# int-brain-lab/mtscomp

Measured on AMD Instinct MI355X. Metric: compress + decompress GB/s (raw int16), higher is better.
Workload: dtype int16

## Files before the change

### mtscomp_amd/csrc/match.hip

```cpp
#include <stdlib.h>

#include <type_traits>

#include "deflate_dev.h"

namespace mts {

__device__ __forceinline__ u32 prev_lane(u32 v, u32 first) { return (u32)__builtin_amdgcn_update_dpp((int)first, (int)v, 0x138, 0xf, 0xf, false); }
__device__ __forceinline__ u32 sel64(u64 mask, u32 a, u32 b)
{
    u32 r;
    asm("v_cndmask_b32_e64 %0, %1, %2, %3" : "=v"(r) : "v"(b), "v"(a), "s"(mask));
    return r;
}
__device__ __forceinline__ u32 and_xor(u32 a, u32 b, u32 c) { return __builtin_amdgcn_bitop3_b32(a, b, c, 0x60); }
__device__ __forceinline__ u64 make_entry(u32 rel, u32 lo, u32 hi)
{
    const u32 d = (((lo >> 5) & 0x3f) << 3) | (lo & 7);
    const u32 w0 = rel | (d << REL_BITS) | (((hi >> 24) & ((1u << (32 - REL_BITS - 9)) - 1)) << (REL_BITS + 9));
    const u32 w1 = (lo >> 24) | (hi << 8);
    return (u64)w0 | ((u64)w1 << 32);
}
__device__ __forceinline__ u32 lds_u32(const u32 *win, u32 addr)
{
    const u32 a = addr >> 2;
    return alignbyte(win[a + 1], win[a], addr & 3);
}

#ifndef MTS_M5_NT_KEYS
#define MTS_M5_NT_KEYS 0
#endif
#ifndef MTS_M5_STATS
#define MTS_M5_STATS 0
#endif
#ifndef MTS_M5_BIT_AND
#define MTS_M5_BIT_AND 0
#endif
#if MTS_M5_STATS
__device__ unsigned long long g_m5_stats[16];
#endif
constexpr int M5_WAVES = 8;
#ifndef MTS_M5_SX
#define MTS_M5_SX 1
#endif
#ifndef MTS_M5_WAVES
#define MTS_M5_WAVES (MTS_M5_SX == 1 ? 8 : MTS_M5_SX == 2 ? 9 : 10)
#endif
constexpr int M5W = MTS_M5_WAVES;
constexpr int M5_SLICES = 64;
constexpr int M6_SLICES = 64;
constexpr int M5_RING = 256;
constexpr int M5_ROWS = 32;
constexpr int M5_LEVELS = 4;
constexpr int M5_ROW_WORDS = M5_RING / 32 + 1;
constexpr int M5_TABLE = M5_ROWS * M5_ROW_WORDS * 4;
constexpr int M5_SLOTS = M5_LEVELS + 1;
constexpr int M5_SX_BYTES = MTS_M5_SX == 1 ? 8 : MTS_M5_SX == 2 ? 4 : 0;
constexpr int M5_WAVE_LDS = M5_RING * (8 + M5_SX_BYTES) + M5_SLOTS * M5_TABLE;
__device__ __forceinline__ constexpr int m5_slot(int d) { return d ? d + 1 : 0; }
#ifndef MTS_M5_LDS_PAD
#define MTS_M5_LDS_PAD 0
#endif
constexpr int M5_VLUT = 129 * 16;
constexpr int MATCH5_LDS = MTS_M5_LDS_PAD ? MTS_M5_LDS_PAD : (M5W * M5_WAVE_LDS + M5_VLUT > 56 * 1024 ? M5W * M5_WAVE_LDS + M5_VLUT : 56 * 1024);

__device__ __forceinline__ int m5_len04(u32 x1, bool &all4)
{
    u32 f;
    asm("v_ffbl_b32 %0, %1" : "=v"(f) : "v"(x1));
    all4 = f > 31;
    return (int)(f >> 3);
}
__device__ __forceinline__ u32 m5_mul24(u32 x, u32 c)
{
    u32 r;
    asm("v_mul_u32_u24 %0, %1, %2" : "=v"(r) : "v"(x), "v"(c));
    return r;
}
__device__ __forceinline__ u32 m5_hash24(u32 x) { return (m5_mul24(x, 0x9E3779u) >> 19) & 31; }
__device__ __forceinline__ u32 m5_ffbh(u32 x)
{
    u32 r;
    asm("v_ffbh_u32 %0, %1" : "=v"(r) : "v"(x));
    return r;
}
__device__ __forceinline__ u32 m5_off8(u32 z, u32 k)
{
    u32 r;
    asm("v_mad_i32_i24 %0, %1, -8, %2" : "=v"(r) : "v"(z), "v"(k));
    return r;
}
__device__ __forceinline__ void m5_keys(u32 e1, u32 (&k)[M5_LEVELS])
{
    const u32 p = m5_mul24(e1, 0x9E3779u);
    k[0] = (p >> 2) & 63;
    k[1] = (p >> 11) & 31;
    k[2] = (p >> 19) & 31;
    k[3] = m5_hash24(e1 ^ (e1 >> 11));
}

__global__ __launch_bounds__(M5W * 64) void k_match5(const u8 *__restrict__ stream, const TileDesc *__restrict__ tiles, int n_tiles, int nsl,
                                                          const u32 *__restrict__ sorted, u32 *__restrict__ tables, u32 *__restrict__ quarter, LevelCfg cfg,
                                                          u32 *__restrict__ flags, int all_quarters)
{
    extern __shared__ __attribute__((aligned(16))) u8 smem[];
    const u32 xcd = blockIdx.x & 7, jb = blockIdx.x >> 3;
    const u32 tile_id = (jb / (u32)nsl) * 8 + xcd, slice = jb % (u32)nsl;
    if (tile_id >= (u32)n_tiles) return;
    const TileDesc td = tiles[tile_id];
    const int wave = threadIdx.x >> 6, lane = threadIdx.x & 63;
    const u8 *gwin = stream + td.stream_off + td.w;
    auto wread = [&](u32 addr) -> u32 { return gld_u32_unaligned(gwin, addr); };
    u64 *SE = (u64 *)(smem + wave * (M5_RING * 8));
    u64 *SX = (u64 *)(smem + M5W * M5_RING * 8 + wave * (M5_RING * 8));
    u32 *TB = (u32 *)(smem + M5W * M5_RING * (8 + M5_SX_BYTES) + M5_VLUT + wave * (M5_SLOTS * M5_TABLE));
    const uint4 *VLUT = (const uint4 *)(smem + M5W * M5_RING * (8 + M5_SX_BYTES));
    typedef __attribute__((address_space(3))) const u64 *lds_u64p;
    const u32 se_base = (u32)(size_t)(__attribute__((address_space(3))) u8 *)(u8 *)SE;
    if (se_base & (M5_RING * 8 - 1)) __builtin_trap();
    auto ring_e = [&](u32 o8) -> u64 { return *(lds_u64p)(size_t)((o8 & (M5_RING * 8 - 8)) | se_base); };
#if MTS_M5_SX == 2
    typedef __attribute__((address_space(3))) const u32 *lds_u32p;
    auto ring_x = [&](u32 o8) -> u32 { return *(lds_u32p)(size_t)((((o8 & (M5_RING * 8 - 8)) | se_base) >> 1) + M5W * M5_RING * 8); };
#else
    auto ring_x = [&](u32 o8) -> u64 { return *(lds_u64p)(size_t)(((o8 & (M5_RING * 8 - 8)) | se_base) + M5W * M5_RING * 8); };
#endif
    u32 *T = tables + td.stream_off, *TQ = quarter + td.stream_off;
    u32 *sink = flags + MATCH_SINK_WORD0 + (blockIdx.x & (MATCH_SINK_LINES - 1)) * MATCH_SINK_LINE_WORDS + (threadIdx.x & 63);
    if (threadIdx.x < 2 && slice == 0) {
        const u32 hashed_end = td.w + td.wlen;
        const u32 p = hashed_end + threadIdx.x;
        if (p >= td.a && p < td.own_end) { T[p] = 0; if (all_quarters) TQ[p] = 0; }
    }
    if (td.wlen == 0) return;
    const u32 *sk = sorted + td.sorted_off;
    const u32 wlen = td.wlen, n = td.n;
    const u32 ngroups = (wlen + 63) / 64;
    const u32 halo = td.a - td.w;
    const u32 chain = (u32)cfg.chain, qchain = (u32)cfg.chain >> 2;
    const u32 nwv = (u32)nsl * M5W;
    const u32 gpw = (ngroups + nwv - 1) / nwv;
    const u32 g_begin = (slice * M5W + wave) * gpw, g_end = min(ngroups, g_begin + gpw);
#if MTS_M5_NT_KEYS
    auto slot_rel = [&](int idx) -> u32 { return __builtin_nontemporal_load(&sk[idx < 0 ? 0 : (u32)idx < wlen ? (u32)idx : wlen - 1]) & REL_MASK; };
#else
    auto slot_rel = [&](int idx) -> u32 { return sk[idx < 0 ? 0 : (u32)idx < wlen ? (u32)idx : wlen - 1] & REL_MASK; };
#endif
#if MTS_M5_NT_KEYS
    auto slot_fwd = [&](u32 idx) -> u32 { return __builtin_nontemporal_load(&sk[min(idx, wlen - 1)]) & REL_MASK; };
#else
    auto slot_fwd = [&](u32 idx) -> u32 { return sk[min(idx, wlen - 1)] & REL_MASK; };
#endif
    const int i_first = (int)g_begin * 64 + lane;
    const u32 r_ha = slot_rel(i_first - 128), r_hb = slot_rel(i_first - 64), r_0 = slot_rel(i_first), r_1 = slot_rel(i_first + 64);
    for (int k = threadIdx.x; k <= 128; k += M5W * 64) {
        uint4 v;
        v.w = k >= 32 ? 0xffffffffu : k ? 0xffffffffu << (32 - k) : 0u;
        v.z = k >= 64 ? 0xffffffffu : k > 32 ? 0xffffffffu << (64 - k) : 0u;
        v.y = k >= 96 ? 0xffffffffu : k > 64 ? 0xffffffffu << (96 - k) : 0u;
        v.x = k >= 128 ? 0xffffffffu : k > 96 ? 0xffffffffu << (128 - k) : 0u;
        ((uint4 *)(smem + M5W * M5_RING * (8 + M5_SX_BYTES)))[k] = v;
    }
    __syncthreads();
    if (g_begin >= g_end) return;
    for (int k = lane; k < M5_SLOTS * M5_TABLE / 16; k += 64) ((uint4 *)TB)[k] = make_uint4(0, 0, 0, 0);
    __builtin_amdgcn_wave_barrier();
    u32 h_carry = 0xffffffffu;
#if MTS_M5_STATS
    u32 st_groups = 0, st_r1 = 0, st_r2 = 0, st_s1 = 0, st_s2 = 0;
    u64 st_t[6] = {0, 0, 0, 0, 0, 0};
    u64 st_mark = 0;
#define M5_MARK(k) do { if (MTS_M5_STATS == 2) { const u64 t_ = (u64)clock64(); st_t[k] += t_ - st_mark; st_mark = t_; } } while (0)
#endif
    u32 rc_carry = 0;
    u32 run_carry = 0;
    const u32 le_lo = lane >= 31 ? 0xffffffffu : (2u << lane) - 1, le_hi = lane < 32 ? 0u : lane == 63 ? 0xffffffffu : (2u << (lane - 32)) - 1;
    u32 inv[6];
#pragma unroll
    for (int j = 0; j < 6; j++) inv[j] = ((lane >> j) & 1) ? 0u : 0xffffffffu;
    auto commit = [&](int idx, u32 rc, u32 lo, u32 hi, u64 x, u32 (&key)[M5_LEVELS], u32 &nbv, u64 &vm) -> u64 {
        const u32 rp = (u32)idx & (M5_RING - 1), word = rp >> 5, bit = 1u << (rp & 31);
        const bool valid = (u32)idx < wlen;
        vm = ballot64(valid);
        const u64 ce = valid ? make_entry(rc, lo, hi) : ~0ull;
        const u32 h = valid ? hash_of(lo) : 0xfffffffeu;
        const u32 hp = prev_lane(h, h_carry), rcp = prev_lane(rc, rc_carry);
        const u64 sr = ballot64(h != hp);
        if (vm & ~sr & ballot64(rc <= rcp)) { if (lane == 0) atomicOr(flags, 1u); }
        h_carry = (u32)__builtin_amdgcn_readlane((int)h, 63);
        rc_carry = (u32)__builtin_amdgcn_readlane((int)rc, 63);
        if (__builtin_popcountll(sr) <= 6) {
            nbv = (u32)lane + run_carry;
            for (u64 m = sr; m; m &= m - 1) { const u32 d = (u32)lane - (u32)__builtin_ctzll(m); nbv = d < nbv ? d : nbv; }
        } else {
            const u32 mlo = (u32)sr & le_lo, mhi = (u32)(sr >> 32) & le_hi;
            const u32 top = mhi ? 63u - (u32)__builtin_clz(mhi) : 31u - (u32)__builtin_clz(mlo | 1u);
            nbv = (mlo | mhi) ? (u32)lane - top : (u32)lane + run_carry;
        }
        nbv = nbv < 128u ? nbv : 128u;
        run_carry = sr ? (u32)__builtin_clzll(sr) + 1u : (run_carry + 64u < 128u ? run_carry + 64u : 128u);
        m5_keys((u32)(ce >> 32), key);
        const u32 wp = word & ~1u;
        {
            u32 *t1 = TB + 2 * (M5_TABLE / 4) + lane * M5_ROW_WORDS + wp;
            t1[0] = 0; t1[1] = 0;
            if (lane < 32) { t1[64 * M5_ROW_WORDS] = 0; t1[64 * M5_ROW_WORDS + 1] = 0; }
            u32 m0 = (u32)vm, m1 = (u32)(vm >> 32);
#pragma unroll
            for (int j = 0; j < 6; j++) {
#if MTS_M5_BIT_AND
                u32 t;
                asm volatile("v_and_b32 %0, %1, %2" : "=v"(t) : "n"(1 << j), "v"(key[0]));
                const u64 B = ballot64(t != 0);
#else
                const u64 B = ballot64((key[0] >> j) & 1);
#endif
                m0 = and_xor(m0, (u32)B, inv[j]); m1 = and_xor(m1, (u32)(B >> 32), inv[j]);
            }
            { u32 *t0 = TB + lane * M5_ROW_WORDS + wp; t0[0] = m0; t0[1] = m1; }
        }
        __builtin_amdgcn_wave_barrier();
#pragma unroll
        for (int d = 1; d < M5_LEVELS; d++)
            if (valid) atomicOr(&TB[m5_slot(d) * (M5_TABLE / 4) + key[d] * M5_ROW_WORDS + word], bit);
        SE[rp] = ce;
#if MTS_M5_SX == 1
        SX[rp] = x;
#elif MTS_M5_SX == 2
        ((u32 *)(smem + M5W * M5_RING * 8))[wave * M5_RING + rp] = (u32)x;
#endif
        return ce;
    };
    typedef u32 u32x4_a4 __attribute__((ext_vector_type(4), aligned(4)));
    auto load16 = [&](u32 r, u32 &lo, u32 &hi, u64 &x) {
        const u8 *q = gwin + (r & ~3u);
        const u32x4_a4 w = *(const u32x4_a4 *)q;
        lo = alignbyte(w.y, w.x, r);
        hi = alignbyte(w.z, w.y, r);
        const u32 b8 = alignbyte(w.w, w.z, r), b12 = alignbyte(0u, w.w, r);
        x = (u64)__builtin_amdgcn_alignbit(b8, hi, 24) | ((u64)(__builtin_amdgcn_alignbit(b12, b8, 24) & 0xffffu) << 32);
    };
    u32 rc_c = r_0, rc_n = r_1;
    u32 lo_c, hi_c;
    u64 x_c;
    {
        u32 kk[M5_LEVELS], nb;
        u64 vmm;
        const u32 ra = r_ha, rb = r_hb;
        u32 la, ha, lb, hb;
        u64 xa, xb;
        load16(ra, la, ha, xa);
        load16(rb, lb, hb, xb);
        load16(rc_c, lo_c, hi_c, x_c);
        *sink = 0;
        commit(i_first - 128, ra, la, ha, xa, kk, nb, vmm);
        __builtin_amdgcn_wave_barrier();
        commit(i_first - 64, rb, lb, hb, xb, kk, nb, vmm);
    }
    for (u32 g = g_begin; g < g_end; g++) {
        const u32 i0 = g * 64, i = i0 + lane;
        u32 key[M5_LEVELS], nbv;
        __builtin_amdgcn_wave_barrier();
#if MTS_M5_STATS == 2
        st_mark = (u64)clock64();
#endif
        u64 vm;
        const u64 e = commit((int)i, rc_c, lo_c, hi_c, x_c, key, nbv, vm);
        const u64 ex = x_c;
        __builtin_amdgcn_wave_barrier();
        rc_c = rc_n;
        load16(rc_c, lo_c, hi_c, x_c);
        rc_n = slot_fwd(i + 128);
        const u32 e0 = (u32)e, e1 = (u32)(e >> 32);
        const u32 rel_p = e0 & REL_MASK;
        const bool own = i < wlen && rel_p >= halo;
        const u64 ownm = vm & ballot64(rel_p >= halo);
#if MTS_M5_STATS == 2
        if (!ownm) { *sink = 0; M5_MARK(5); continue; }
        M5_MARK(0);
#else
        if (!ownm) { *sink = 0; continue; }
#endif
        const u32 p_abs = td.w + rel_p;
        const u32 look = n - p_abs;
        const u32 maxlen = look < (u32)MAX_MATCH ? look : (u32)MAX_MATCH;
        const u32 nice = (u32)cfg.nice < look ? (u32)cfg.nice : look;
        const int lim1 = (int)(p_abs > (u32)MAX_DIST + 1 ? p_abs - MAX_DIST - 1 : 0) - (int)td.w;
        const int limn = (int)(p_abs > (u32)MAX_DIST ? p_abs - MAX_DIST : 0) - (int)td.w;
        const u32 lo = (i + 128) & (M5_RING - 1), w0 = lo >> 5, sh = lo & 31, lo8 = lo << 3;
        nbv = own ? (nbv < chain ? nbv : chain) : 0;
        u32 V[4], A4[4], A5[4], A6[4], A7[4];
        {
            const uint4 v = VLUT[nbv];
            V[0] = v.x; V[1] = v.y; V[2] = v.z; V[3] = v.w;
        }
        auto rowmask = [&](const int d, const u32 (&in)[4], u32 (&out)[4]) __attribute__((always_inline)) {
            const u8 *row = (const u8 *)(TB + m5_slot(d) * (M5_TABLE / 4) + key[d] * M5_ROW_WORDS);
            auto word = [&](const u32 k) -> u32 { return *(const u32 *)(row + (((w0 + k) << 2) & 28u)); };
            const u32 W0 = word(0), W1 = word(1), W2 = word(2), W3 = word(3), W4 = word(4);
            out[0] = in[0] & __builtin_amdgcn_alignbit(W1, W0, sh);
            out[1] = in[1] & __builtin_amdgcn_alignbit(W2, W1, sh);
            out[2] = in[2] & __builtin_amdgcn_alignbit(W3, W2, sh);
            out[3] = in[3] & __builtin_amdgcn_alignbit(W4, W3, sh);
        };
        rowmask(0, V, A4);
        rowmask(1, A4, A5);
        rowmask(2, A5, A6);
        rowmask(3, A6, A7);
#if MTS_M5_STATS == 2
        asm volatile("" :: "v"(A7[0]), "v"(A7[1]), "v"(A7[2]), "v"(A7[3]));
        M5_MARK(1);
#endif
        int best = -1, qbest = -1;
        u32 bdist = 0, qdist = 0;
        asm volatile("" : "+v"(best), "+v"(bdist));
        auto walks = [&](auto near_end) __attribute__((always_inline)) {
        constexpr bool NEAR_END = decltype(near_end)::value;
        auto set_stop = [&]() {
#pragma unroll
            for (int w = 0; w < 4; w++) { A4[w] = 0; A5[w] = 0; A6[w] = 0; A7[w] = 0; }
        };
        auto cand = [&](const u32 o8 , const u32 c0, const u32 c1, const u32 rel_c, auto &&narrow, auto &&finish) __attribute__((always_inline)) {
            const u32 x0 = (c0 ^ e0) >> REL_BITS, x1 = c1 ^ e1;
            if ((x0 & 0x1ff) == 0) {
                bool all4;
                int len = m5_len04(x1, all4);
                if (all4) len = 4;
                if (all4 && (x0 >> 9) == 0) {
#if MTS_M5_SX == 1
                    const u64 y = ring_x(o8) ^ ex;
                    const u32 len0 = 13;
#elif MTS_M5_SX == 2
                    const u32 y = ring_x(o8) ^ (u32)ex;
                    const u32 len0 = 11;
#else
                    const u32 y = wread(rel_c + 7) ^ (u32)ex;
                    const u32 len0 = 11;
#endif
                    if (y) len = 4 + (int)((u32)__builtin_ctzll((u64)y) >> 3);
                    else {
                        const u32 cap = NEAR_END ? maxlen : (u32)MAX_MATCH;
                        u32 full = len0;
                        while (full < cap) {
                            const u32 x = wread(rel_c + full) ^ wread(rel_p + full);
                            if (x) { full += (u32)__builtin_ctz(x) >> 3; break; }
                            full += 4;
                        }
                        full = full < cap ? full : cap;
                        len = (int)full - 3;
                        if (!NEAR_END && full >= (u32)cfg.nice) { best = len; bdist = rel_p - rel_c; set_stop(); finish(); }
                    }
                }
                if (NEAR_END) len = len < (int)maxlen - 3 ? len : (int)maxlen - 3;
                if (len > best) {
                    best = len; bdist = rel_p - rel_c;
                    narrow();
                    if (NEAR_END && len >= (int)nice - 3) { set_stop(); finish(); }
                }
            }
        };
        auto walk = [&](const u32 tb, const u32 &m0, const u32 &m1, const u32 &m2, const u32 &m3, const u32 &m4, const u32 part, const bool head) __attribute__((always_inline)) {
            auto pick = [&]() -> u32 {
                u32 r = best >= 0 ? m1 : m0;
                asm volatile("" : "+v"(r));
                r = best >= 1 ? m2 : r;
                asm volatile("" : "+v"(r));
                r = best >= 2 ? m3 : r;
                asm volatile("" : "+v"(r));
                return best >= 3 ? m4 : r;
            };
            auto pick_longer = [&]() -> u32 {
                u32 r = best >= 1 ? m2 : m1;
                asm volatile("" : "+v"(r));
                r = best >= 2 ? m3 : r;
                asm volatile("" : "+v"(r));
                return best >= 3 ? m4 : r;
            };
            u32 el = head ? m0 & part : pick() & part;
            if (head) {
#if MTS_M5_STATS
                st_r1++; st_s1 += (u32)__popcll(ballot64(el != 0));
#endif
                const u32 o8 = lo8 + 127 * 8;
                const u64 c = ring_e(o8);
                if ((int)el < 0) {
                    el &= 0x7fffffffu;
                    const u32 c0 = (u32)c, c1 = (u32)(c >> 32);
                    const u32 rel_c = c0 & REL_MASK;
                    if ((int)rel_c > lim1) cand(o8, c0, c1, rel_c, [&]() { el &= pick_longer(); }, [&]() { el = 0; });
                    else el = 0;
                }
            }
            while (any64(el != 0)) {
#if MTS_M5_STATS
                st_r1++; st_s1 += (u32)__popcll(ballot64(el != 0));
#endif
                {
                    const bool had = el != 0;
                    const u32 z = m5_ffbh(el);
                    const u32 t = tb + 31 - z;
                    const u32 o8 = m5_off8(z, lo8 + ((tb + 31) << 3));
                    const u64 c = ring_e(o8);
                    const u32 c0 = (u32)c, c1 = (u32)(c >> 32);
                    const u32 rel_c = c0 & REL_MASK;
                    const bool in_range = had && (int)rel_c > ((!head && t == 127) ? lim1 : limn);
                    u32 rm = in_range ? 0xffffffffu : 0u;
                    asm volatile("" : "+v"(rm));
                    el = el & ~(0x80000000u >> (z & 31)) & rm;
                    if (in_range) cand(o8, c0, c1, rel_c, [&]() { el &= pick_longer(); }, [&]() { el = 0; });
                }
            }
        };
        const u32 qpart = qchain >= 32 ? 0xffffffffu : ~(0xffffffffu >> qchain);
#define MTS_WALK(w, part, head) walk(32 * (w), V[w], A4[w], A5[w], A6[w], A7[w], part, head)
        MTS_WALK(3, qpart, true);
        qbest = best; qdist = bdist;
        if (qpart != 0xffffffffu) MTS_WALK(3, ~qpart, false);
#undef MTS_WALK
#if MTS_M5_STATS == 2
        M5_MARK(2);
#endif
        {
            auto pickw = [&](const int w) __attribute__((always_inline)) -> u32 {
                u32 r = best >= 1 ? A5[w] : A4[w];
                asm volatile("" : "+v"(r));
                r = best >= 2 ? A6[w] : r;
                asm volatile("" : "+v"(r));
                return best >= 3 ? A7[w] : r;
            };
            const u64 c3 = ballot64(best >= 0), c4 = ballot64(best >= 1), c5 = ballot64(best >= 2), c6 = ballot64(best >= 3);
            auto pick0 = [&](const int w) __attribute__((always_inline)) -> u32 {
                u32 r = sel64(c3, A4[w], V[w]);
                r = sel64(c4, A5[w], r);
                r = sel64(c5, A6[w], r);
                return sel64(c6, A7[w], r);
            };
            u32 f2 = pick0(2), f1 = pick0(1), f0 = pick0(0);
            u32 ko2 = lo8 + ((64 + 31) << 3), ko1 = lo8 + ((32 + 31) << 3), ko0 = lo8 + (31 << 3);
            asm volatile("" : "+v"(ko2), "+v"(ko1), "+v"(ko0));
            while (any64((f2 | f1 | f0) != 0)) {
#if MTS_M5_STATS
                st_r2++; st_s2 += (u32)__popcll(ballot64((f2 | f1 | f0) != 0));
#endif
                if (f2 | f1 | f0) {
                    const bool t2 = f2 != 0, t1 = f1 != 0;
                    const u32 cur = t2 ? f2 : t1 ? f1 : f0;
                    const u32 tbo = t2 ? ko2 : t1 ? ko1 : ko0;
                    const u32 z = (u32)__builtin_clz(cur);
                    const u32 o8 = m5_off8(z, tbo);
                    const u64 c = ring_e(o8);
                    const u32 c0 = (u32)c, c1 = (u32)(c >> 32);
                    const u32 rel_c = c0 & REL_MASK;
                    const bool in_range = (int)rel_c > limn;
                    u32 rm = in_range ? 0xffffffffu : 0u;
                    asm volatile("" : "+v"(rm));
                    const u32 ncur = cur & ~(0x80000000u >> z);
                    f2 = (t2 ? ncur : f2) & rm;
                    f1 = ((!t2 && t1) ? ncur : f1) & rm;
                    f0 = ((!t2 && !t1) ? ncur : f0) & rm;
                    if (in_range) cand(o8, c0, c1, rel_c, [&]() { f2 &= pickw(2); f1 &= pickw(1); f0 &= pickw(0); }, [&]() { f2 = 0; f1 = 0; f0 = 0; });
                }
            }
        }
        };
        if (ownm & ballot64(look < (u32)MAX_MATCH)) walks(std::true_type{}); else walks(std::false_type{});
#if MTS_M5_STATS == 2
        M5_MARK(3);
#endif
        {
            const u32 f = bdist | ((u32)(best > 0 ? best : 0) << 15), q = qdist | ((u32)(qbest > 0 ? qbest : 0) << 15);
            u32 e = f;
            const bool differ = q != f, side = differ && qbest > (int)cfg.good - 3;
            if (differ) e |= side ? TE_QSIDE : TE_QNONE;
            if (own && (side || all_quarters)) TQ[p_abs] = q;
            u32 *dst = own ? T + p_abs : sink;
            *dst = e;
        }
#if MTS_M5_STATS
        st_groups++;
#if MTS_M5_STATS == 2
        M5_MARK(4);
#endif
#endif
    }
#if MTS_M5_STATS
    if (lane == 0) { atomicAdd(&g_m5_stats[0], st_groups); atomicAdd(&g_m5_stats[1], st_r1); atomicAdd(&g_m5_stats[2], st_r2); atomicAdd(&g_m5_stats[3], st_s1); atomicAdd(&g_m5_stats[4], st_s2); for (int k = 0; k < 6; k++) atomicAdd(&g_m5_stats[5 + k], st_t[k]); }
#endif
}

constexpr int M6_RING = 1024;
constexpr int M6_ROW_WORDS = M6_RING / 32 + 1;
constexpr int M6_TABLE = M5_ROWS * M6_ROW_WORDS * 4;
constexpr int MATCH6_LDS = 2 * M6_RING * 8 + M5_SLOTS * M6_TABLE + M5_VLUT;

__global__ __launch_bounds__(M5_WAVES * 64) void k_match6(const u8 *__restrict__ stream, const TileDesc *__restrict__ tiles, int n_tiles, int nsl,
                                                          const u32 *__restrict__ sorted, u32 *__restrict__ tables, u32 *__restrict__ quarter, LevelCfg cfg,
                                                          u32 *__restrict__ flags, int all_quarters)
{
    extern __shared__ __attribute__((aligned(16))) u8 smem[];
    __shared__ u32 wg_h[M5_WAVES], wg_rc[M5_WAVES], wg_tail[M5_WAVES], wg_min;
    const u32 xcd = blockIdx.x & 7, jb = blockIdx.x >> 3;
    const u32 tile_id = (jb / (u32)nsl) * 8 + xcd, slice = jb % (u32)nsl;
    if (tile_id >= (u32)n_tiles) return;
    const TileDesc td = tiles[tile_id];
    const int wave = threadIdx.x >> 6, lane = threadIdx.x & 63;
    const u8 *gwin = stream + td.stream_off + td.w;
    auto wread = [&](u32 addr) -> u32 { return gld_u32_unaligned(gwin, addr); };
    u64 *SE = (u64 *)smem;
    u64 *SX = SE + M6_RING;
    u32 *TB = (u32 *)(smem + 2 * M6_RING * 8);
    u32 *T = tables + td.stream_off, *TQ = quarter + td.stream_off;
    if (threadIdx.x < 2 && slice == 0) {
        const u32 hashed_end = td.w + td.wlen;
        const u32 p = hashed_end + threadIdx.x;
        if (p >= td.a && p < td.own_end) { T[p] = 0; if (all_quarters) TQ[p] = 0; }
    }
    if (td.wlen == 0) return;
    const u32 *sk = sorted + td.sorted_off;
    const u32 wlen = td.wlen, n = td.n;
    const u32 ngroups = (wlen + 63) / 64;
    const u32 halo = td.a - td.w;
    const u32 chain = (u32)cfg.chain, qchain = (u32)cfg.chain >> 2;
    const u32 gpb = ((ngroups + (u32)nsl - 1) / (u32)nsl + M5_WAVES - 1) / M5_WAVES * M5_WAVES;
    const u32 gb_begin = slice * gpb, gb_end = min(ngroups, gb_begin + gpb);
    if (gb_begin >= gb_end) return;
    for (int k = threadIdx.x; k < M5_SLOTS * M6_TABLE / 4; k += M5_WAVES * 64) TB[k] = 0;
    const uint4 *VLUT = (const uint4 *)(smem + 2 * M6_RING * 8 + M5_SLOTS * M6_TABLE);
    for (int k = threadIdx.x; k <= 128; k += M5_WAVES * 64) {
        uint4 v;
        v.w = k >= 32 ? 0xffffffffu : k ? 0xffffffffu << (32 - k) : 0u;
        v.z = k >= 64 ? 0xffffffffu : k > 32 ? 0xffffffffu << (64 - k) : 0u;
        v.y = k >= 96 ? 0xffffffffu : k > 64 ? 0xffffffffu << (96 - k) : 0u;
        v.x = k >= 128 ? 0xffffffffu : k > 96 ? 0xffffffffu << (128 - k) : 0u;
        ((uint4 *)(smem + 2 * M6_RING * 8 + M5_SLOTS * M6_TABLE))[k] = v;
    }
    u32 inv[6];
#pragma unroll
    for (int j = 0; j < 6; j++) inv[j] = ((lane >> j) & 1) ? 0u : 0xffffffffu;
    typedef u32 u32x4_a4 __attribute__((ext_vector_type(4), aligned(4)));
    auto load16 = [&](u32 r, u32 &lo, u32 &hi, u64 &x) {
        const u8 *q = gwin + (r & ~3u);
        const u32x4_a4 w = *(const u32x4_a4 *)q;
        lo = alignbyte(w.y, w.x, r);
        hi = alignbyte(w.z, w.y, r);
        const u32 b8 = alignbyte(w.w, w.z, r), b12 = alignbyte(0u, w.w, r) & 0xffu;
        x = (u64)(hi >> 24) | ((u64)b8 << 8) | ((u64)b12 << 40);
    };
    struct Batch { bool valid; u32 rc, lo, hi; u64 x; };
    auto fetch = [&](int idx0, Batch &bt) {
        const int idx = idx0 + lane;
        bt.valid = idx >= 0 && (u32)idx < wlen;
        bt.rc = bt.valid ? sk[idx] & REL_MASK : 0;
        load16(bt.rc, bt.lo, bt.hi, bt.x);
    };
    auto commit = [&](int idx0, const Batch &bt) {
        const u32 rp = (u32)(idx0 + lane) & (M6_RING - 1), word = rp >> 5, bit = 1u << (rp & 31);
        const u64 ce = bt.valid ? make_entry(bt.rc, bt.lo, bt.hi) : ~0ull;
        u32 key[M5_LEVELS];
        m5_keys((u32)(ce >> 32), key);
        const u32 wp = word & ~1u;
        u32 *t1 = TB + 2 * (M6_TABLE / 4) + lane * M6_ROW_WORDS + wp;
        t1[0] = 0; t1[1] = 0;
        if (lane < 32) { t1[64 * M6_ROW_WORDS] = 0; t1[64 * M6_ROW_WORDS + 1] = 0; }
        const u64 vm = ballot64(bt.valid);
        u32 m0 = (u32)vm, m1 = (u32)(vm >> 32);
#pragma unroll
        for (int j = 0; j < 6; j++) {
            const u64 B = ballot64((key[0] >> j) & 1);
            m0 = and_xor(m0, (u32)B, inv[j]); m1 = and_xor(m1, (u32)(B >> 32), inv[j]);
        }
        { u32 *t0 = TB + lane * M6_ROW_WORDS + wp; t0[0] = m0; t0[1] = m1; }
        __builtin_amdgcn_wave_barrier();
#pragma unroll
        for (int d = 1; d < M5_LEVELS; d++)
            if (bt.valid) atomicOr(&TB[m5_slot(d) * (M6_TABLE / 4) + key[d] * M6_ROW_WORDS + word], bit);
        SE[rp] = ce;
        SX[rp] = bt.x;
    };
    u32 c_h = 0xfffffffdu, c_rc = 0, c_tail = 0;
    if (gb_begin > 0) {
        const u32 i1 = gb_begin * 64 - 1;
        c_rc = sk[i1] & REL_MASK;
        c_h = hash_of(wread(c_rc));
        if (threadIdx.x == 0) wg_min = 0xffffffffu;
        __syncthreads();
        for (u32 r = 0; r * (M5_WAVES * 64) < chain; r++) {
            const u32 t = 1 + threadIdx.x + r * (M5_WAVES * 64);
            const bool mism = t > i1 || hash_of(wread(sk[i1 - (t > i1 ? 0 : t)] & REL_MASK)) != c_h;
            if (mism) atomicMin(&wg_min, t);
            __syncthreads();
            const u32 found = wg_min;
            __syncthreads();
            if (found != 0xffffffffu) break;
        }
        c_tail = wg_min < chain ? wg_min : chain;
        __syncthreads();
    }
    for (u32 gs = gb_begin; gs < gb_end; gs += M5_WAVES) {
        const int G0 = (int)gs * 64;
        const u32 g = gs + (u32)wave;
        const bool active = g < gb_end;
        const u32 i = g * 64 + lane;
        const u32 rp0 = (active && i < wlen) ? sk[i] & REL_MASK : 0;
        u32 own_lo, own_hi;
        u64 ex;
        load16(rp0, own_lo, own_hi, ex);
        Batch ba, bb;
        fetch(G0 - 128 + 64 * wave, ba);
        if (wave < 2) fetch(G0 - 128 + 64 * (wave + 8), bb);
        const u64 e = make_entry(rp0, own_lo, own_hi);
        const u32 e0 = (u32)e, e1 = (u32)(e >> 32);
        const u32 rel_p = e0 & REL_MASK;
        const bool own = active && i < wlen && rel_p >= halo;
        u32 key[M5_LEVELS];
        m5_keys(e1, key);
        const u32 p_abs = td.w + rel_p;
        const u32 look = n - p_abs;
        const u32 maxlen = look < (u32)MAX_MATCH ? look : (u32)MAX_MATCH;
        const u32 nice = (u32)cfg.nice < look ? (u32)cfg.nice : look;
        const int lim1 = (int)(p_abs > (u32)MAX_DIST + 1 ? p_abs - MAX_DIST - 1 : 0) - (int)td.w;
        const int limn = (int)(p_abs > (u32)MAX_DIST ? p_abs - MAX_DIST : 0) - (int)td.w;
        u32 best = 2, bdist = 0, qbest = 2, qdist = 0;
        bool stop = false, qtaken = false;
        const bool have = active && i < wlen;
        const u32 h_own = have ? hash_of(own_lo) : 0xfffffffeu;
        if (lane == 63) { wg_h[wave] = h_own; wg_rc[wave] = rel_p; }
        __syncthreads();
        commit(G0 - 128 + 64 * wave, ba);
        if (wave < 2) commit(G0 - 128 + 64 * (wave + 8), bb);
        u32 nbv;
        {
            u32 hp = __shfl_up(h_own, 1, 64), rcp = __shfl_up(rel_p, 1, 64);
            if (lane == 0) { hp = wave ? wg_h[wave - 1] : c_h; rcp = wave ? wg_rc[wave - 1] : c_rc; }
            const bool starts_run = h_own != hp;
            if (any64(have && !starts_run && rel_p <= rcp)) { if (lane == 0) atomicOr(flags, 1u); }
            const u64 sr = ballot64(starts_run);
            if (lane == 0) wg_tail[wave] = sr ? (u32)__builtin_clzll(sr) + 1u : 0u;
            __syncthreads();
            u32 t = c_tail;
            for (int w = 0; w < wave; w++) { const u32 x = wg_tail[w]; t = x ? x : (t + 64u < chain ? t + 64u : chain); }
            const u32 le_lo = lane >= 31 ? 0xffffffffu : (2u << lane) - 1, le_hi = lane < 32 ? 0u : lane == 63 ? 0xffffffffu : (2u << (lane - 32)) - 1;
            const u32 mlo = (u32)sr & le_lo, mhi = (u32)(sr >> 32) & le_hi;
            const u32 top = mhi ? 63u - (u32)__builtin_clz(mhi) : 31u - (u32)__builtin_clz(mlo | 1u);
            nbv = (mlo | mhi) ? (u32)lane - top : (u32)lane + t;
            nbv = own ? (nbv < chain ? nbv : chain) : 0;
            u32 tt = c_tail;
            for (int w = 0; w < M5_WAVES; w++) { const u32 x = wg_tail[w]; tt = x ? x : (tt + 64u < chain ? tt + 64u : chain); }
            c_tail = tt; c_h = wg_h[M5_WAVES - 1]; c_rc = wg_rc[M5_WAVES - 1];
        }
        if (wave < 2) fetch(G0 - 256 + 64 * wave, ba);
        for (u32 jbase = 0, blk = 0;; jbase += 128, blk++) {
            if ((u32)(wave >> 1) == (blk & 3)) commit(G0 - (int)jbase - 256 + 64 * (wave & 1), ba);
            if ((u32)(wave >> 1) == ((blk + 1) & 3)) fetch(G0 - (int)jbase - 384 + 64 * (wave & 1), ba);
            if (jbase == qchain && !qtaken) { qbest = best; qdist = bdist; qtaken = true; }
            const u32 nbl = nbv > jbase ? (nbv - jbase < 128 ? nbv - jbase : 128) : 0;
            if (any64(nbl != 0 && !stop)) {
                const u32 lo = (u32)((int)i - (int)jbase - 128) & (M6_RING - 1), w0 = lo >> 5, sh = lo & 31;
                u32 V[4], A4[4], A5[4], A6[4], A7[4];
                {
                    const uint4 v = VLUT[nbl];
                    V[0] = v.x; V[1] = v.y; V[2] = v.z; V[3] = v.w;
                }
                auto rowmask = [&](const int d, const u32 (&in)[4], u32 (&out)[4]) __attribute__((always_inline)) {
                    const u8 *row = (const u8 *)(TB + m5_slot(d) * (M6_TABLE / 4) + key[d] * M6_ROW_WORDS);
                    auto word = [&](const u32 k) -> u32 { return *(const u32 *)(row + (((w0 + k) << 2) & 124u)); };
                    const u32 W0 = word(0), W1 = word(1), W2 = word(2), W3 = word(3), W4 = word(4);
                    out[0] = in[0] & __builtin_amdgcn_alignbit(W1, W0, sh);
                    out[1] = in[1] & __builtin_amdgcn_alignbit(W2, W1, sh);
                    out[2] = in[2] & __builtin_amdgcn_alignbit(W3, W2, sh);
                    out[3] = in[3] & __builtin_amdgcn_alignbit(W4, W3, sh);
                };
                rowmask(0, V, A4);
                rowmask(1, A4, A5);
                rowmask(2, A5, A6);
                rowmask(3, A6, A7);
                auto pickw = [&](const int w) __attribute__((always_inline)) -> u32 {
                    u32 r = best >= 3 ? A4[w] : V[w];
                    asm volatile("" : "+v"(r));
                    r = best >= 4 ? A5[w] : r;
                    asm volatile("" : "+v"(r));
                    r = best >= 5 ? A6[w] : r;
                    asm volatile("" : "+v"(r));
                    return best >= 6 ? A7[w] : r;
                };
                const bool first = jbase == 0;
                auto walk = [&](const bool u3, const bool u2, const bool u1, const bool u0) __attribute__((always_inline)) {
                    u32 f3 = (stop || !u3) ? 0u : pickw(3), f2 = (stop || !u2) ? 0u : pickw(2);
                    u32 f1 = (stop || !u1) ? 0u : pickw(1), f0 = (stop || !u0) ? 0u : pickw(0);
                    while (any64((f3 | f2 | f1 | f0) != 0)) {
                        if (f3 | f2 | f1 | f0) {
                            const bool t3 = f3 != 0, t2 = f2 != 0, t1 = f1 != 0;
                            const u32 cur = t3 ? f3 : t2 ? f2 : t1 ? f1 : f0;
                            const u32 tb = t3 ? 96u : t2 ? 64u : t1 ? 32u : 0u;
                            const u32 z = (u32)__builtin_clz(cur);
                            const u32 ncur = cur & ~(0x80000000u >> z);
                            f3 = t3 ? ncur : f3;
                            f2 = (!t3 && t2) ? ncur : f2;
                            f1 = (!t3 && !t2 && t1) ? ncur : f1;
                            f0 = (!t3 && !t2 && !t1) ? ncur : f0;
                            const u32 t = tb + 31 - z;
                            const u32 slot = (lo + t) & (M6_RING - 1);
                            const u64 c = SE[slot];
                            const u32 c0 = (u32)c, c1 = (u32)(c >> 32);
                            const u32 rel_c = c0 & REL_MASK;
                            if ((int)rel_c > ((first && t == 127) ? lim1 : limn)) {
                                const u32 x0 = (c0 ^ e0) >> REL_BITS, x1 = c1 ^ e1;
                                if ((x0 & 0x1ff) == 0) {
                                    u32 len = x1 ? 3 + ((u32)__builtin_ctz(x1) >> 3) : 7;
                                    if (x1 == 0 && (x0 >> 9) == 0) {
                                        const u64 y = SX[slot] ^ ex;
                                        if (y) len = 7 + ((u32)__builtin_ctzll(y) >> 3);
                                        else {
                                            len = 13;
                                            while (len < maxlen) {
                                                const u32 x = wread(rel_c + len) ^ wread(rel_p + len);
                                                if (x) { len += (u32)__builtin_ctz(x) >> 3; break; }
                                                len += 4;
                                            }
                                        }
                                    }
                                    len = len < maxlen ? len : maxlen;
                                    if (len > best) {
                                        best = len; bdist = rel_p - rel_c;
                                        if (len >= nice) stop = true;
                                        f3 &= pickw(3); f2 &= pickw(2); f1 &= pickw(1); f0 &= pickw(0);
                                    }
                                }
                            } else stop = true;
                            if (stop) { f3 = 0; f2 = 0; f1 = 0; f0 = 0; }
                        }
                    }
                };
                if (first && qchain == 64) {
                    walk(true, true, false, false);
                    qbest = best; qdist = bdist; qtaken = true;
                    walk(false, false, true, true);
                } else walk(true, true, true, true);
            } else if (jbase == 0 && qchain == 64) { qbest = best; qdist = bdist; qtaken = true; }
            if (!__syncthreads_or(!stop && nbv > jbase + 128)) break;
        }
        if (!qtaken) { qbest = best; qdist = bdist; }
        if (own) te_store(T, TQ, p_abs, best, bdist, qbest, qdist, (u32)cfg.good, all_quarters);
    }
}

int launch_match(hipStream_t st, const u8 *d_stream, const TileDesc *d_tiles, int n_tiles, const u32 *d_sorted, u32 *d_tables, u32 *d_quarter,
                 LevelCfg cfg, u32 *d_flags, int all_quarters)
{
    if (n_tiles == 0) return MTS_OK;
    if (cfg.chain <= 128) {
        if (MATCH5_LDS > 65536) MTS_LDS_ATTR(k_match5, MATCH5_LDS);
        int nsl = M5_SLICES;
        if (const char *e = getenv("MTS_MATCH_SLICES")) nsl = atoi(e) > 0 ? atoi(e) : nsl;
        const int grid = (n_tiles + 7) / 8 * 8 * nsl;
        hipLaunchKernelGGL(k_match5, dim3(grid), dim3(M5W * 64), MATCH5_LDS, st, d_stream, d_tiles, n_tiles, nsl, d_sorted, d_tables, d_quarter, cfg, d_flags, all_quarters);
    } else {
        if (cfg.chain != 256 && (cfg.chain >> 2) % 128 != 0) { set_error("match: chain budget %d unsupported", cfg.chain); return MTS_E_INTERNAL; }
        const int nsl = M6_SLICES;
        const int grid = (n_tiles + 7) / 8 * 8 * nsl;
        hipLaunchKernelGGL(k_match6, dim3(grid), dim3(M5_WAVES * 64), MATCH6_LDS, st, d_stream, d_tiles, n_tiles, nsl, d_sorted, d_tables, d_quarter, cfg, d_flags, all_quarters);
    }
    MTS_HIP(hipGetLastError());
    return MTS_OK;
}

}

#if MTS_M5_STATS
extern "C" int mts_debug_m5_stats(unsigned long long *out)
{
    if (hipMemcpyFromSymbol(out, HIP_SYMBOL(mts::g_m5_stats), 128) != hipSuccess) return -1;
    unsigned long long z[16] = {0};
    return hipMemcpyToSymbol(HIP_SYMBOL(mts::g_m5_stats), z, 128) == hipSuccess ? 0 : -1;
}
#endif
```

Measured before the change: 35.67.

## Specialize match5 commit and rowmask on ring phase with precomputed LDS addresses

Result: faster. 36.23 (median of 6 runs) (+1.6%).

```diff
diff --git a/mtscomp_amd/csrc/match.hip b/mtscomp_amd/csrc/match.hip
--- a/mtscomp_amd/csrc/match.hip
+++ b/mtscomp_amd/csrc/match.hip
@@ -112,7 +112,6 @@
     const u8 *gwin = stream + td.stream_off + td.w;
     auto wread = [&](u32 addr) -> u32 { return gld_u32_unaligned(gwin, addr); };
     u64 *SE = (u64 *)(smem + wave * (M5_RING * 8));
-    u64 *SX = (u64 *)(smem + M5W * M5_RING * 8 + wave * (M5_RING * 8));
     u32 *TB = (u32 *)(smem + M5W * M5_RING * (8 + M5_SX_BYTES) + M5_VLUT + wave * (M5_SLOTS * M5_TABLE));
     const uint4 *VLUT = (const uint4 *)(smem + M5W * M5_RING * (8 + M5_SX_BYTES));
     typedef __attribute__((address_space(3))) const u64 *lds_u64p;
@@ -178,10 +177,22 @@
     u32 inv[6];
 #pragma unroll
     for (int j = 0; j < 6; j++) inv[j] = ((lane >> j) & 1) ? 0u : 0xffffffffu;
-    auto commit = [&](int idx, u32 rc, u32 lo, u32 hi, u64 x, u32 (&key)[M5_LEVELS], u32 &nbv, u64 &vm) -> u64 {
-        const u32 rp = (u32)idx & (M5_RING - 1), word = rp >> 5, bit = 1u << (rp & 31);
-        const bool valid = (u32)idx < wlen;
-        vm = ballot64(valid);
+    typedef __attribute__((address_space(3))) u32 *lds_w32p;
+    typedef __attribute__((address_space(3))) u64 *lds_w64p;
+    auto lds32 = [](u32 a) -> lds_w32p { return (lds_w32p)(size_t)a; };
+    auto lds64 = [](u32 a) -> lds_w64p { return (lds_w64p)(size_t)a; };
+    const u32 tb_base = (u32)(size_t)(__attribute__((address_space(3))) u8 *)(u8 *)TB;
+    u32 a_ring = se_base + (u32)lane * 8;
+    u32 a_row0 = tb_base + (u32)lane * (M5_ROW_WORDS * 4);
+    u32 a_row1 = a_row0 + 2 * M5_TABLE;
+    u32 a_row2 = a_row1 + 64 * (M5_ROW_WORDS * 4);
+    u32 a_tab0 = tb_base + ((u32)lane >> 5) * 4, a_tab1 = a_tab0 + m5_slot(1) * M5_TABLE, a_tab2 = a_tab0 + m5_slot(2) * M5_TABLE, a_tab3 = a_tab0 + m5_slot(3) * M5_TABLE;
+    auto a_tab = [&](const int d) __attribute__((always_inline)) -> u32 { return d == 0 ? a_tab0 : d == 1 ? a_tab1 : d == 2 ? a_tab2 : a_tab3; };
+    const u32 lane_bit = 1u << (lane & 31), lane_sh = (u32)lane & 31;
+    const bool lower = lane < 32;
+    auto commit = [&](auto phase, const bool valid, const u64 vm, u32 rc, u32 lo, u32 hi, u64 x, u32 (&key)[M5_LEVELS], u32 &nbv) __attribute__((always_inline)) -> u64 {
+        constexpr u32 PH = decltype(phase)::value;
+        constexpr u32 WP = 2 * PH;
         const u64 ce = valid ? make_entry(rc, lo, hi) : ~0ull;
         const u32 h = valid ? hash_of(lo) : 0xfffffffeu;
         const u32 hp = prev_lane(h, h_carry), rcp = prev_lane(rc, rc_carry);
@@ -200,11 +211,11 @@
         nbv = nbv < 128u ? nbv : 128u;
         run_carry = sr ? (u32)__builtin_clzll(sr) + 1u : (run_carry + 64u < 128u ? run_carry + 64u : 128u);
         m5_keys((u32)(ce >> 32), key);
-        const u32 wp = word & ~1u;
         {
-            u32 *t1 = TB + 2 * (M5_TABLE / 4) + lane * M5_ROW_WORDS + wp;
+            lds_w32p t1 = lds32(a_row1 + WP * 4), t2 = lds32(a_row2 + WP * 4);
             t1[0] = 0; t1[1] = 0;
-            if (lane < 32) { t1[64 * M5_ROW_WORDS] = 0; t1[64 * M5_ROW_WORDS + 1] = 0; }
+            if (PH == 0) t1[8] = 0;
+            if (lower) { t2[0] = 0; t2[1] = 0; if (PH == 0) t2[8] = 0; }
             u32 m0 = (u32)vm, m1 = (u32)(vm >> 32);
 #pragma unroll
             for (int j = 0; j < 6; j++) {
@@ -217,35 +228,50 @@
 #endif
                 m0 = and_xor(m0, (u32)B, inv[j]); m1 = and_xor(m1, (u32)(B >> 32), inv[j]);
             }
-            { u32 *t0 = TB + lane * M5_ROW_WORDS + wp; t0[0] = m0; t0[1] = m1; }
+            { lds_w32p t0 = lds32(a_row0 + WP * 4); t0[0] = m0; t0[1] = m1; if (PH == 0) t0[8] = m0; }
         }
         __builtin_amdgcn_wave_barrier();
 #pragma unroll
         for (int d = 1; d < M5_LEVELS; d++)
-            if (valid) atomicOr(&TB[m5_slot(d) * (M5_TABLE / 4) + key[d] * M5_ROW_WORDS + word], bit);
-        SE[rp] = ce;
+            if (valid) __hip_atomic_fetch_or(lds32(key[d] * (M5_ROW_WORDS * 4) + a_tab(d) + WP * 4), lane_bit, __ATOMIC_RELAXED, __HIP_MEMORY_SCOPE_AGENT);
+        if (PH == 0) {
+#pragma unroll
+            for (int d = 1; d < M5_LEVELS; d++)
+                if (valid && lower) __hip_atomic_fetch_or(lds32(key[d] * (M5_ROW_WORDS * 4) + a_tab(d) + 8 * 4), lane_bit, __ATOMIC_RELAXED, __HIP_MEMORY_SCOPE_AGENT);
+        }
+        *lds64(a_ring + PH * 512) = ce;
 #if MTS_M5_SX == 1
-        SX[rp] = x;
+        *lds64(a_ring + (M5W * M5_RING * 8 + PH * 512)) = x;
 #elif MTS_M5_SX == 2
-        ((u32 *)(smem + M5W * M5_RING * 8))[wave * M5_RING + rp] = (u32)x;
+        *lds32((a_ring >> 1) + (M5W * M5_RING * 8 + PH * 256)) = (u32)x;
 #endif
         return ce;
     };
+    auto by_phase = [&](u32 ph, auto &&f) __attribute__((always_inline)) {
+        switch (ph) {
+        case 0: return f(std::integral_constant<u32, 0>{});
+        case 1: return f(std::integral_constant<u32, 1>{});
+        case 2: return f(std::integral_constant<u32, 2>{});
+        default: return f(std::integral_constant<u32, 3>{});
+        }
+    };
     typedef u32 u32x4_a4 __attribute__((ext_vector_type(4), aligned(4)));
-    auto load16 = [&](u32 r, u32 &lo, u32 &hi, u64 &x) {
-        const u8 *q = gwin + (r & ~3u);
-        const u32x4_a4 w = *(const u32x4_a4 *)q;
+    auto fetch16 = [&](u32 r) -> u32x4_a4 { return *(const u32x4_a4 *)(gwin + (r & ~3u)); };
+    auto unpack16 = [&](const u32x4_a4 w, u32 r, u32 &lo, u32 &hi, u64 &x) {
         lo = alignbyte(w.y, w.x, r);
         hi = alignbyte(w.z, w.y, r);
         const u32 b8 = alignbyte(w.w, w.z, r), b12 = alignbyte(0u, w.w, r);
         x = (u64)__builtin_amdgcn_alignbit(b8, hi, 24) | ((u64)(__builtin_amdgcn_alignbit(b12, b8, 24) & 0xffffu) << 32);
     };
+    auto load16 = [&](u32 r, u32 &lo, u32 &hi, u64 &x) { unpack16(fetch16(r), r, lo, hi, x); };
+    u32 ph = (u32)__builtin_amdgcn_readfirstlane((int)(g_begin & 3));
     u32 rc_c = r_0, rc_n = r_1;
     u32 lo_c, hi_c;
     u64 x_c;
     {
         u32 kk[M5_LEVELS], nb;
-        u64 vmm;
+        const bool va = (u32)(i_first - 128) < wlen, vb = (u32)(i_first - 64) < wlen;
+        const u64 vma = ballot64(va), vmb = ballot64(vb);
         const u32 ra = r_ha, rb = r_hb;
         u32 la, ha, lb, hb;
         u64 xa, xb;
@@ -253,33 +279,68 @@
         load16(rb, lb, hb, xb);
         load16(rc_c, lo_c, hi_c, x_c);
         *sink = 0;
-        commit(i_first - 128, ra, la, ha, xa, kk, nb, vmm);
+        by_phase(ph ^ 2, [&](auto phase) { commit(phase, va, vma, ra, la, ha, xa, kk, nb); });
         __builtin_amdgcn_wave_barrier();
-        commit(i_first - 64, rb, lb, hb, xb, kk, nb, vmm);
+        by_phase((ph + 3) & 3, [&](auto phase) { commit(phase, vb, vmb, rb, lb, hb, xb, kk, nb); });
     }
-    for (u32 g = g_begin; g < g_end; g++) {
+    for (u32 g = g_begin; g < g_end; g++, ph = (ph + 1) & 3) {
         const u32 i0 = g * 64, i = i0 + lane;
         u32 key[M5_LEVELS], nbv;
+        asm volatile("" : "+v"(a_ring), "+v"(a_row0), "+v"(a_row1), "+v"(a_row2), "+v"(a_tab0), "+v"(a_tab1), "+v"(a_tab2), "+v"(a_tab3));
         __builtin_amdgcn_wave_barrier();
 #if MTS_M5_STATS == 2
         st_mark = (u64)clock64();
 #endif
-        u64 vm;
-        const u64 e = commit((int)i, rc_c, lo_c, hi_c, x_c, key, nbv, vm);
-        const u64 ex = x_c;
-        __builtin_amdgcn_wave_barrier();
-        rc_c = rc_n;
-        load16(rc_c, lo_c, hi_c, x_c);
-        rc_n = slot_fwd(i + 128);
-        const u32 e0 = (u32)e, e1 = (u32)(e >> 32);
-        const u32 rel_p = e0 & REL_MASK;
-        const bool own = i < wlen && rel_p >= halo;
-        const u64 ownm = vm & ballot64(rel_p >= halo);
+        const bool valid = i < wlen;
+        const u64 vm = ballot64(valid);
+        u64 e, ex, ownm;
+        u32x4_a4 w_n;
+        auto next_bytes = [&]() __attribute__((always_inline)) { unpack16(w_n, rc_c, lo_c, hi_c, x_c); };
+        u32 e0, e1, rel_p, lo8;
+        bool own;
+        u32 V[4], A4[4], A5[4], A6[4], A7[4];
+        auto front = [&](auto phase) __attribute__((always_inline)) -> bool {
+            constexpr u32 PH = decltype(phase)::value;
+            e = commit(phase, valid, vm, rc_c, lo_c, hi_c, x_c, key, nbv);
+            ex = x_c;
+            __builtin_amdgcn_wave_barrier();
+            rc_c = rc_n;
+            w_n = fetch16(rc_c);
+            rc_n = slot_fwd(i + 128);
+            e0 = (u32)e; e1 = (u32)(e >> 32);
+            rel_p = e0 & REL_MASK;
+            own = valid && rel_p >= halo;
+            ownm = vm & ballot64(rel_p >= halo);
+            if (!ownm) return false;
 #if MTS_M5_STATS == 2
-        if (!ownm) { *sink = 0; M5_MARK(5); continue; }
-        M5_MARK(0);
+            M5_MARK(0);
+#endif
+            constexpr u32 PL = (PH + 2) & 3, W = 2 * PL;
+            lo8 = a_ring + PL * 512;
+            nbv = own ? (nbv < chain ? nbv : chain) : 0;
+            {
+                const uint4 v = VLUT[nbv];
+                V[0] = v.x; V[1] = v.y; V[2] = v.z; V[3] = v.w;
+            }
+            auto rowmask = [&](const int d, const u32 (&in)[4], u32 (&out)[4]) __attribute__((always_inline)) {
+                const u32 row = key[d] * (M5_ROW_WORDS * 4) + a_tab(d);
+                auto word = [&](const u32 k) -> u32 { return *lds32(row + ((W + k) & 7) * 4); };
+                const u32 W0 = word(0), W1 = word(1), W2 = word(2), W3 = word(3), W4 = word(4);
+                out[0] = in[0] & __builtin_amdgcn_alignbit(W1, W0, lane_sh);
+                out[1] = in[1] & __builtin_amdgcn_alignbit(W2, W1, lane_sh);
+                out[2] = in[2] & __builtin_amdgcn_alignbit(W3, W2, lane_sh);
+                out[3] = in[3] & __builtin_amdgcn_alignbit(W4, W3, lane_sh);
+            };
+            rowmask(0, V, A4);
+            rowmask(1, A4, A5);
+            rowmask(2, A5, A6);
+            rowmask(3, A6, A7);
+            return true;
+        };
+#if MTS_M5_STATS == 2
+        if (!by_phase(ph, front)) { *sink = 0; next_bytes(); M5_MARK(5); continue; }
 #else
-        if (!ownm) { *sink = 0; continue; }
+        if (!by_phase(ph, front)) { *sink = 0; next_bytes(); continue; }
 #endif
         const u32 p_abs = td.w + rel_p;
         const u32 look = n - p_abs;
@@ -287,26 +348,6 @@
         const u32 nice = (u32)cfg.nice < look ? (u32)cfg.nice : look;
         const int lim1 = (int)(p_abs > (u32)MAX_DIST + 1 ? p_abs - MAX_DIST - 1 : 0) - (int)td.w;
         const int limn = (int)(p_abs > (u32)MAX_DIST ? p_abs - MAX_DIST : 0) - (int)td.w;
-        const u32 lo = (i + 128) & (M5_RING - 1), w0 = lo >> 5, sh = lo & 31, lo8 = lo << 3;
-        nbv = own ? (nbv < chain ? nbv : chain) : 0;
-        u32 V[4], A4[4], A5[4], A6[4], A7[4];
-        {
-            const uint4 v = VLUT[nbv];
-            V[0] = v.x; V[1] = v.y; V[2] = v.z; V[3] = v.w;
-        }
-        auto rowmask = [&](const int d, const u32 (&in)[4], u32 (&out)[4]) __attribute__((always_inline)) {
-            const u8 *row = (const u8 *)(TB + m5_slot(d) * (M5_TABLE / 4) + key[d] * M5_ROW_WORDS);
-            auto word = [&](const u32 k) -> u32 { return *(const u32 *)(row + (((w0 + k) << 2) & 28u)); };
-            const u32 W0 = word(0), W1 = word(1), W2 = word(2), W3 = word(3), W4 = word(4);
-            out[0] = in[0] & __builtin_amdgcn_alignbit(W1, W0, sh);
-            out[1] = in[1] & __builtin_amdgcn_alignbit(W2, W1, sh);
-            out[2] = in[2] & __builtin_amdgcn_alignbit(W3, W2, sh);
-            out[3] = in[3] & __builtin_amdgcn_alignbit(W4, W3, sh);
-        };
-        rowmask(0, V, A4);
-        rowmask(1, A4, A5);
-        rowmask(2, A5, A6);
-        rowmask(3, A6, A7);
 #if MTS_M5_STATS == 2
         asm volatile("" :: "v"(A7[0]), "v"(A7[1]), "v"(A7[2]), "v"(A7[3]));
         M5_MARK(1);
@@ -476,6 +517,7 @@
             u32 *dst = own ? T + p_abs : sink;
             *dst = e;
         }
+        next_bytes();
 #if MTS_M5_STATS
         st_groups++;
 #if MTS_M5_STATS == 2
```
